# dpmerrell/PathMatFac.jl

Measured on AMD Instinct MI355X. Metric: fit_iters_per_sec, higher is better.
Workload: dtype f32; 1 GPU; fit! epoch on synthetic 200000x50000 matrix (D stored as f32), K=64, Gaussian loss, group-reg X (32 groups) + featureset-ARD Y, adam; rows sharded over 1 GPU(s); full_model=False, M=200000, N=50000, K=64, rows_per_gpu=200000, optimizer=adam, parallelism=single GPU, rccl_ranks=0, collectives_issued=0, column_chunks=1

## Files before the change

### pathmatfac.jl_amd/csrc/pmf_common.h

```cpp
#ifndef PMF_COMMON_H
#define PMF_COMMON_H
#include <hip/hip_runtime.h>

#include <cstdint>
#include <type_traits>
#include <unordered_map>

#include "../../include/pmf_hip.h"

int pmf_fail(const char *fmt, ...);
#define HIPCHK(x)                                                                                    \
  do {                                                                                               \
    hipError_t e_ = (x);                                                                             \
    if (e_ != hipSuccess) return pmf_fail("%s failed: %s (%s:%d)", #x, hipGetErrorString(e_), __FILE__, __LINE__); \
  } while (0)
#define PMFCHK(x)          \
  do {                     \
    int r_ = (x);          \
    if (r_ < 0) return r_; \
  } while (0)

typedef std::unordered_map<const void *, size_t> PmfDynLds;
int pmf_ensure_dyn_lds(PmfDynLds *cache, const void *kern, size_t lds);

// ... 42 lines not shown
  int32_t nbs_shift;
  int32_t n_bv;
  double *loss_partial;
  int64_t M, N;
  int32_t n_cseg;
  int32_t want_gx, want_gy;
  unsigned long long *stamps;
  int32_t dbg;
  const ViewDesc *views;
  const char *Xsb, *Ysb;
  int32_t ct0;
  float *gx_part;
  const int32_t *piece_base;
  int64_t gx_slot_stride;
  const float *sb_scale_x, *sb_scale_y;
};

__device__ __forceinline__ int pmf_rowmap(int r, int h) { return (r & 3) + 8 * (r >> 2) + 4 * h; }
__device__ __forceinline__ bool pmf_finite(float y) { return fabsf(y) <= 3.402823466e38f; }

__host__ __device__ __forceinline__ int pmf_meta_kind(int meta) { return meta & 3; }
__host__ __device__ __forceinline__ int pmf_meta_view(int meta) { return (meta >> 2) - 1; }
__host__ __device__ __forceinline__ int64_t pmf_view_index(const ViewDesc &vd, int64_t j, int b) { return (j - vd.c0) * vd.nb + b; }
__host__ __device__ __forceinline__ int64_t pmf_btab_index(const ViewDesc &vd, int64_t j, int b) { return vd.tab_off + pmf_view_index(vd, j, b); }
__device__ __forceinline__ int pmf_row_batch(const int32_t *bor, int64_t M, int v, int64_t i) { return v >= 0 ? bor[(int64_t)v * M + i] : -1; }
__device__ __forceinline__ float2 pmf_batch_dt(const ViewDesc &vd, const float2 *btab, int64_t j, int b) {
  return b >= 0 ? btab[pmf_btab_index(vd, j, b)] : make_float2(1.f, 0.f);
}

__device__ __forceinline__ void pmf_noise(int kind, float z, float y, float w, float &l, float &g) {
// ... 294 lines not shown
```

### pathmatfac.jl_amd/csrc/pmf_ctx.h

```cpp
#ifndef PMF_CTX_H
#define PMF_CTX_H
#include <hip/hip_runtime.h>

#include <algorithm>
#include <chrono>
#include <cmath>
#include <cstdarg>
#include <cstdio>
#include <cstdlib>
#include <cstring>
#include <string>
#include <unordered_map>
#include <vector>

#include "pmf_common.h"

struct ParamBuf {
  float *p = nullptr, *g = nullptr, *acc = nullptr, *mom = nullptr;
  float *wq = nullptr, *cq = nullptr;
  float *wl1 = nullptr;
  int64_t n = 0;
  float bp1 = 0.f, bp2 = 0.f;
};

// ... 42 lines not shown
  int64_t n = 0, V = 0;
  float p = 1.f;
  std::vector<int64_t> h_voff;
  int64_t *voff = nullptr;
  int64_t *aa_rp = nullptr, *ab_rp = nullptr, *abt_rp = nullptr, *bb_rp = nullptr;
  int32_t *aa_col = nullptr, *ab_col = nullptr, *abt_col = nullptr, *bb_col = nullptr;
  float *aa_val = nullptr, *ab_val = nullptr, *abt_val = nullptr, *bb_val = nullptr;
  float *u = nullptr;
  float *work = nullptr;
  float *PT = nullptr;
  float *grad = nullptr;
  int32_t *iters = nullptr;
  double *uloss = nullptr;
  int rb = 1;
  int64_t vmax = 0;
};

struct pmf_ctx {
  int device = 0;
  hipStream_t stream = nullptr;
  bool own_stream = true;
  int n_cu = 256;
  int64_t M = 0, N = 0;
  int K = 0, Kp = 0, KB = 0;
  void *D = nullptr;
  bool own_D = false;
  int64_t D_M = 0, D_Npad = 0, nRB = 0;
  uint32_t *tflags = nullptr;
  int64_t tflags_cap = 0;
  bool tflags_valid = false;
// ... 39 lines not shown
  std::vector<uint8_t> h_kind;
  std::vector<int64_t> noise_s1, noise_e1;
  std::vector<WorkSplit> splits;
  int n_chunks_req = 0;
  float *gx_part = nullptr;
  size_t gx_part_cap = 0;
  int32_t *gx_off = nullptr, *gx_idx = nullptr;
  int64_t gx_serial = -1;
  int64_t split_serial = 0;
  Comm comm;
  int last_chunks = 1;
  hipEvent_t ev_host = nullptr;
  int64_t kind_version = 0;
  float *gy_slabs = nullptr;
  size_t gy_slabs_cap = 0;
  int precision = PMF_PREC_F32;
  char *xsb = nullptr, *ysb = nullptr;
  size_t xsb_cap = 0, ysb_cap = 0;
  float *sb8_scale = nullptr;
  uint32_t *sb8_max = nullptr;
  int64_t sb_launches = 0;
  int64_t loss_cap = 0;
  int64_t n_macro = 0;
  double *reg_partial = nullptr;
  double *d_loss = nullptr;
  double *h_loss = nullptr;
  std::vector<std::pair<hipEvent_t, hipEvent_t>> ev_pool;
  size_t ev_used = 0;
  double kernel_ms_sum = 0.0;
  int64_t kernel_launches = 0;
// ... 30 lines not shown
    HIPCHK(hipFree(*p));
    *p = nullptr;
  }
  if (n == 0) n = 1;
  HIPCHK(hipMalloc((void **)p, n * sizeof(T)));
  if (zero) PMFCHK(memset_now(*p, 0, n * sizeof(T)));
  return 0;
}
template <typename T>
static void dev_free(T **p) {
  if (*p) (void)hipFree(*p);
  *p = nullptr;
}

template <typename T>
struct DevBuf {
  T *p = nullptr;
  DevBuf() = default;
  DevBuf(const DevBuf &) = delete;
  DevBuf &operator=(const DevBuf &) = delete;
  ~DevBuf() { if (p) (void)hipFree(p); }
  int alloc(size_t n) {
    HIPCHK(hipMalloc((void **)&p, std::max<size_t>(n, 1) * sizeof(T)));
    return 0;
  }
};
template <typename T>
struct PinnedBuf {
  T *p = nullptr;
  PinnedBuf() = default;
  PinnedBuf(const PinnedBuf &) = delete;
  PinnedBuf &operator=(const PinnedBuf &) = delete;
  ~PinnedBuf() { if (p) (void)hipHostFree(p); }
  int alloc(size_t n) {
    HIPCHK(hipHostMalloc((void **)&p, std::max<size_t>(n, 1) * sizeof(T)));
    return 0;
  }
};

__device__ __forceinline__ double block_reduce_sum(double v, double *sh) {
#pragma unroll
  for (int off = 32; off > 0; off >>= 1) v += __shfl_xor(v, off, 64);
// ... 29 lines not shown
  const float b = 1.f + (0.5f / be) * (p * p);
  lacc += (double)(scale * (0.5f + al) * logf(b));
  g += scale * ((al + 0.5f) * p / (b * be));
}

int ctx_bind(pmf_ctx *c);
int ensure_dyn_lds(pmf_ctx *c, const void *kern, size_t lds);
int check_ready(pmf_ctx *c);
int harvest_events(pmf_ctx *c);
int epoch_open(pmf_ctx *c, const pmf_fit_opts *o);
int epoch_layer_pass(pmf_ctx *c, const pmf_fit_opts *o, bool with_loss);
FusedGeom fused_geometry(pmf_ctx *c, bool want_gx, bool want_gy, bool allow_chunks);
int prepare_fused_pass(pmf_ctx *c, const FusedGeom &g, bool want_gx, bool want_gy);
int launch_fused_chunk(pmf_ctx *c, const FusedGeom &g, int s, bool want_gx, bool want_gy);
struct PassExtent { const char *name; int64_t need, cap; };
constexpr int PMF_PASS_EXTENTS = 10;
int fused_pass_extents(pmf_ctx *c, const FusedGeom &g, bool want_gx, bool want_gy, PassExtent *out);
int check_pass_extents(const PassExtent *e, int n);
int guard_fused_pass(pmf_ctx *c, const FusedGeom &g, bool want_gx, bool want_gy);
int step_param_range(pmf_ctx *c, int which, int64_t e0, int64_t n, bool do_step, bool use_reg, int reg_slot, int *reg_count,
                     int max_blocks, bool advance);
int step_param(pmf_ctx *c, int which, bool do_step, bool use_reg, int reg_slot, int *reg_count);
int step_layers(pmf_ctx *c, const pmf_fit_opts *o, int *reg_count);
int launch_loss_reduce(pmf_ctx *c, const RegCounts &rc, int mask);
void step_args_xy(pmf_ctx *c, int which, StepArgs *s);
int eval_full_loss(pmf_ctx *c, double out[4]);
int eval_data_grads(pmf_ctx *c);
int stats_pass_check(pmf_ctx *c);
int stats_pass(pmf_ctx *c, int use_factors, bool want_cols, bool want_batch, const float **cols, const float **batch);
void lbfgs_free(pmf_ctx *c);
void netreg_free(pmf_ctx *c, int which);
// ... 7 lines not shown
```

### pathmatfac.jl_amd/csrc/pmf_fused.hip.inc

```

template <int KB, int NW, int RBW = 1>
struct FusedCfg {
  static constexpr int Kp = 32 * KB;
  static constexpr int KpS = Kp + 4;
  static constexpr int SLAB = 32 * Kp;
  static constexpr int YT = PMF_BN * KpS;
  static constexpr int XP = 32 * KpS;
  static constexpr int TT = (RBW - 1) * 1024;
  static constexpr int FIXED = NW * SLAB + NW * RBW * XP + NW * TT + 8 * PMF_BN + 4;
  static constexpr int LDS_BUDGET = 160 * 1024;
  static constexpr int NYB = (2 * YT + FIXED) * 4 + 8 * NW <= LDS_BUDGET ? 2 : 1;
  static constexpr size_t lds_bytes = (sizeof(float) * (NYB * YT + FIXED) + sizeof(double) * NW + 15) / 16 * 16;
  static constexpr size_t lds_batch_extra = PMF_BN * 16 * sizeof(float2) + PMF_PM_BYTES + NW * RBW * 16 * 32;
};

#ifndef PMF_NW4_WAVES
#define PMF_NW4_WAVES 1
#endif
template <int KB, int NW, int RBW, int BMODE, bool MIXED, int GM, bool DB, bool XW = false>
__global__ __launch_bounds__(64 * NW, (NW == 8 ? 2 : PMF_NW4_WAVES)) void pmf_fused_kernel(const FusedArgs a) {
  using Cfg = FusedCfg<KB, NW, RBW>;
  constexpr bool FULL = GM != 3;
  constexpr bool BATCH = BMODE != 0;
  constexpr bool bt_lds = BMODE == 1;
// ... 43 lines not shown
  }
  const int xw_j = 16 * (w & 1) + (lane & 15), xw_k = 16 * (w >> 1) + 4 * (lane >> 4);
  const int xw_e = xw_j * Kp + xw_k;
  const int xw_x = 4 * (lane >> 4) * KpS + 16 * (w >> 1) + (lane & 15);
  int xw_g[4];
  typedef const __attribute__((address_space(3))) float *lds_cptr;
  unsigned xw_xa[4];
#pragma unroll
  for (int u = 0; u < 4; ++u) {
    const int i = 4 * (lane >> 4) + u;
    xw_g[u] = i * 32 + 4 * ((xw_j >> 2) ^ (i & 7)) + (xw_j & 3);
    xw_xa[u] = (unsigned)(uintptr_t)(lds_cptr)(Xs + xw_x + u * KpS);
    if (XW) asm volatile("" : "+v"(xw_xa[u]));
  }

  constexpr bool HOIST = KB == 2 && NW == 8 && RBW == 1 && GM != 3 && (XW || GM != 0 || BMODE == 0);
  unsigned ho_y[2][YV], ho_s[2][YV], ho_c[2], ho_g[2][RV4];
  if (HOIST) {
#pragma unroll
    for (int z = 0; z < 2; ++z) {
      const int ncol = z == 0 || N % BN == 0 ? BN : (int)(N % BN);
#pragma unroll
      for (int q = 0; q < YV; ++q) {
        int e4 = tid + NT * q;
        if (e4 > BN * Kp / 4 - 1) e4 = BN * Kp / 4 - 1;
        int jl = (e4 * 4) / Kp;
        if (jl >= ncol) { jl = ncol - 1; e4 = jl * (Kp / 4); }
        ho_y[z][q] = 16u * e4;
        ho_s[z][q] = 16u * jl;
        asm volatile("" : "+v"(ho_y[z][q]), "+v"(ho_s[z][q]));
      }
      ho_c[z] = 16u * (tid < ncol ? tid : ncol - 1);
      asm volatile("" : "+v"(ho_c[z]));
#pragma unroll
      for (int q = 0; q < RV4; ++q) {
        int e = xw_e;
        if (!XW) {
          const int f = tid + NT * q, ff = f < BN * Kp / 4 ? f : 0;
          e = ((ff % (BN * 8)) / 8) * Kp + 32 * (ff / (BN * 8)) + 4 * (ff % 8);
        }
        ho_g[z][q] = 4u * (e < ncol * Kp ? e : e % Kp);
        asm volatile("" : "+v"(ho_g[z][q]));
      }
    }
  }
  auto ho_at = [](const void *base, unsigned off) { return reinterpret_cast<const char *>(base) + off; };
#ifdef PMF_STAMPS
  unsigned long long st_acc[16] = {0, 0, 0, 0, 0, 0, 0, 0, 0, 0, 0, 0, 0, 0, 0, 0};
  unsigned long long st_prev = __builtin_amdgcn_s_memtime();
  const unsigned long long st_t0 = st_prev, st_r0 = __builtin_amdgcn_s_memrealtime();
#endif
  const int wg = pmf_xcd_wg(blockIdx.x, gridDim.x);
  const int64_t w_begin = a.wg_begin[wg];
  const int64_t w_end = a.wg_begin[wg + 1];
  float *myslab = a.gy_slabs + (int64_t)wg * a.slab_stride;
  const int64_t seg_block = a.n_rp * a.tps;
  double lossacc = 0.0;
  int seg_cur = -1, pidx = 0, t0_first = 0;
  int gx_slot = (GM == 2) ? 0 : a.piece_base[wg];
// ... 27 lines not shown
      for (int q = 0; q < XV; ++q) {
        const int e4 = lane + 64 * q;
        const int il = (e4 * 4) / Kp;
        const int64_t ir = row0[rb] + il < M ? row0[rb] + il : M - 1;
        xv0[rb][q] = *reinterpret_cast<const float4 *>(a.X + ir * Kp + (e4 * 4) % Kp);
      }
    }
    f32x16 gx[RBW][KB];
#pragma unroll
    for (int rb = 0; rb < RBW; ++rb)
#pragma unroll
      for (int kb = 0; kb < KB; ++kb)
#pragma unroll
        for (int r = 0; r < 16; ++r) gx[rb][kb][r] = 0.f;

    auto stage_load_y = [&](int64_t jt, int q, float4 (&yv)[YV], float (&sgv)[YV]) {
      const float *yb = a.Y + jt * Kp;
      const float4 *cb = a.colp + jt;
      const int64_t rem = N - jt;
      if (HOIST) {
        const bool rag = rem < BN;
        yv[q] = *reinterpret_cast<const float4 *>(ho_at(yb, rag ? ho_y[1][q] : ho_y[0][q]));
        sgv[q] = *reinterpret_cast<const float *>(ho_at(cb, rag ? ho_s[1][q] : ho_s[0][q]));
        return;
      }
      const int ncol = rem > BN ? BN : (int)rem;
      int e4 = tid + NT * q;
      if (e4 > BN * Kp / 4 - 1) e4 = BN * Kp / 4 - 1;
      int jl = (e4 * 4) / Kp;
      if (jl >= ncol) { jl = ncol - 1; e4 = jl * (Kp / 4); }
      yv[q] = *reinterpret_cast<const float4 *>(yb + e4 * 4);
      sgv[q] = cb[jl].x;
    };
    auto stage_load_c = [&](int64_t jt, float4 &cv) {
      const float4 *cb = a.colp + jt;
      const int64_t rem = N - jt;
      if (HOIST) {
        cv = *reinterpret_cast<const float4 *>(ho_at(cb, rem < BN ? ho_c[1] : ho_c[0]));
        return;
      }
      const int ncol = rem > BN ? BN : (int)rem;
      cv = cb[tid < ncol ? tid : ncol - 1];
    };
    auto stage_load = [&](int64_t jt, float4 (&yv)[YV], float (&sgv)[YV], float4 &cv) {
#pragma unroll
      for (int q = 0; q < YV; ++q) stage_load_y(jt, q, yv, sgv);
      stage_load_c(jt, cv);
    };
    auto stage_store = [&](int ybuf, int cbuf, int64_t jt, const float4 (&yv)[YV], const float (&sgv)[YV], const float4 &cv) {
      float *Yn = Ys + ybuf * Cfg::YT;
      const int64_t rem = N - jt;
      const int ncol = rem > BN ? BN : (int)rem;
#pragma unroll
      for (int q = 0; q < YV; ++q) {
        const int e4 = tid + NT * q;
        if (e4 < BN * Kp / 4) {
          const int jl = (e4 * 4) / Kp, kf = (e4 * 4) % Kp;
          const float sg = jl < ncol ? sgv[q] : 0.f;
          *reinterpret_cast<float4 *>(Yn + jl * KpS + kf) = make_float4(yv[q].x * sg, yv[q].y * sg, yv[q].z * sg, yv[q].w * sg);
        }
      }
      asm volatile("" ::"v"(cv.x), "v"(cv.y), "v"(cv.z), "v"(cv.w));
      if (tid < BN) {
        const bool livec = tid < ncol;
        Csg[cbuf * BN + tid] = livec ? cv.x : 0.f;
        Cmu[cbuf * BN + tid] = livec ? cv.y : 0.f;
        Cw[cbuf * BN + tid] = livec ? cv.z : 0.f;
        Cmt[cbuf * BN + tid] = livec ? __float_as_int(cv.w) : 3;
        if (MIXED) {
          const int kd = __float_as_int(cv.w) & 3;
          const unsigned m0 = (unsigned)__ballot(!livec || kd == 0), m1 = (unsigned)__ballot(!livec || kd == 1),
                         m2 = (unsigned)__ballot(!livec || kd == 2);
          if (tid == 0) Ck[cbuf] = m0 == 0xffffffffu ? 0 : (m1 == 0xffffffffu ? 1 : (m2 == 0xffffffffu ? 2 : 3));
        }
        if (bt_lds) {
          const int vw = (__float_as_int(cv.w) >> 2) - 1;
          const int vw0 = __builtin_amdgcn_readfirstlane(vw);
          const unsigned mv = (unsigned)__ballot(!livec || vw == vw0);
          if (tid == 0) Ck[2 + cbuf] = mv == 0xffffffffu ? vw0 : -2;
        }
      }
    };
    auto bt_e = [&](int q) { return (tid & 31) * 16 + (tid >> 5) + (NT / 32) * q; };
// ... 3 lines not shown
      Btd[o] = dt.x;
      Btt[o] = dt.y + mu;
    };
    float4 gold[RV4];
    PmfDTile<DB> dcur[RBW];
    constexpr int DCH = PmfDTile<DB>::NCH;
    auto slab_map = [&](int q, int &so, int &e) -> bool {
      const int f = tid + NT * q;
      const bool in = f < BN * Kp / 4;
      const int ff = in ? f : 0;
      so = 4 * ff;
      e = ((ff % (BN * 8)) / 8) * Kp + 32 * (ff / (BN * 8)) + 4 * (ff % 8);
      return in;
    };
    auto slab_prefetch_one = [&](int64_t jt, int q) {
      const float *sb = myslab + jt * Kp;
      const int64_t rem = N - jt;
      if (HOIST) {
        gold[q] = pmf_load_stream(reinterpret_cast<const float4 *>(ho_at(sb, rem < BN ? ho_g[1][q] : ho_g[0][q])));
        return;
      }
      const int nel = (rem > BN ? BN : (int)rem) * Kp;
      int so, e;
      if (XW) e = xw_e;
      else slab_map(q, so, e);
      gold[q] = pmf_load_stream(reinterpret_cast<const float4 *>(sb + (e < nel ? e : (e % Kp))));
    };
    auto forward_reduce = [&](f32x16 (&acc)[RBW], int ybuf, int cbuf, bool do_red, int64_t jt_red) {
      const int cb0 = cbuf * BN + 4 * h;
#pragma unroll
      for (int r = 0; r < 16; ++r) {
        const float m0 = BATCH ? 0.f : Cmu[cb0 + (r & 3) + 8 * (r >> 2)];
#pragma unroll
        for (int rb = 0; rb < RBW; ++rb) acc[rb][r] = m0;
      }
      const float4 *yr = reinterpret_cast<const float4 *>(Ys + ybuf * Cfg::YT + l31 * KpS + h * (Kp / 2));
      const float4 *xr[RBW];
      float4 yv = yr[0], xv[RBW];
#pragma unroll
      for (int rb = 0; rb < RBW; ++rb) {
        xr[rb] = reinterpret_cast<const float4 *>(Xw[rb] + l31 * KpS + h * (Kp / 2));
// ... 35 lines not shown
        for (int rb = 0; rb < RBW; ++rb) acc[rb] = __builtin_amdgcn_mfma_f32_32x32x2f32(yv.y, xv[rb].y, acc[rb], 0, 0, 0);
#pragma unroll
        for (int rb = 0; rb < RBW; ++rb) acc[rb] = __builtin_amdgcn_mfma_f32_32x32x2f32(yv.z, xv[rb].z, acc[rb], 0, 0, 0);
#pragma unroll
        for (int rb = 0; rb < RBW; ++rb) acc[rb] = __builtin_amdgcn_mfma_f32_32x32x2f32(yv.w, xv[rb].w, acc[rb], 0, 0, 0);
        yv = yn;
#pragma unroll
        for (int rb = 0; rb < RBW; ++rb) xv[rb] = xn[rb];
        __builtin_amdgcn_sched_barrier(0);
      }
      if (do_red && (FULL || !(dbg & 8))) {
#pragma unroll
        for (int rb = 0; rb < RBW; ++rb) {
          dcur[rb].touch();
        }
        const int64_t rem = N - jt_red;
        const int nel = (rem > BN ? BN : (int)rem) * Kp;
        float *sb = myslab + jt_red * Kp;
#pragma unroll
        for (int q = 0; q < RV4; ++q) {
          float4 v = racc[q];
          const float sgj = Csg[(cbuf ^ 1) * BN + eo[q] / Kp];
          v.x *= sgj; v.y *= sgj; v.z *= sgj; v.w *= sgj;
          if (!slab_first) { v.x += gold[q].x; v.y += gold[q].y; v.z += gold[q].z; v.w += gold[q].w; }
          if (in[q] && eo[q] < nel) pmf_store_stream(reinterpret_cast<float4 *>(sb + eo[q]), v);
        }
      }
    };

    bool rows_in[RBW];
    int rb_u[RBW];
    uint32_t tflag[RBW];
#pragma unroll
    for (int rb = 0; rb < RBW; ++rb) {
      const int rb_raw = __builtin_amdgcn_readfirstlane((int)(row0[rb] >> 5));
      rows_in[rb] = rb_raw < a.nRB;
      rb_u[rb] = rows_in[rb] ? rb_raw : (int)a.nRB - 1;
      tflag[rb] = a.tflags[(col_begin >> 5) * a.nRB + rb_u[rb]];
#pragma unroll
      for (int q = 0; q < DCH; ++q) dcur[rb].load(a.D, (col_begin >> 5) * a.nRB + rb_u[rb], lane, q);
    }
    {
      float4 yv[YV], cv;
      float sgv[YV];
      stage_load(col_begin, yv, sgv, cv);
#pragma unroll
      for (int rb = 0; rb < RBW; ++rb)
#pragma unroll
        for (int q = 0; q < XV; ++q) {
          const int e4 = lane + 64 * q;
          const int il = (e4 * 4) / Kp, kf = (e4 * 4) % Kp;
          *reinterpret_cast<float4 *>(Xw[rb] + il * KpS + kf) = row0[rb] + il < M ? xv0[rb][q] : make_float4(0.f, 0.f, 0.f, 0.f);
        }
      stage_store(0, 0, col_begin, yv, sgv, cv);
      if (bt_lds) {
#pragma unroll
        for (int q = 0; q < NBT; ++q) {
          const int e = bt_e(q);
          bt_store(e, pmf_bt_entry(a, a.pm + rp * a.n_bv * 16, col_begin, e, pmf_bt_view(a, col_begin, e)), bt_mu(col_begin, e));
        }
        if (tid < a.n_bv * 16) Pm[tid] = a.pm[rp * a.n_bv * 16 + tid];
        if (h == 0)
#pragma unroll
          for (int rb = 0; rb < RBW; ++rb)
            for (int v = 0; v < a.n_bv; ++v) Bw0[rb * 512 + v * 32 + l31] = a.row_slot[(int64_t)v * M + irow_c[rb]];
      }
    }
    __syncthreads();

    f32x16 acc[RBW];
    forward_reduce(acc, 0, 0, false, 0);

    for (int t = 0; t < ntiles; ++t) {
      const int par = t & 1;
      const int cur = NYB == 2 ? par : 0, nxt = NYB == 2 ? (par ^ 1) : 0;
      const int64_t j0 = col_begin + (int64_t)t * BN;
      const float *Yc = Ys + cur * Cfg::YT;
      const bool have_next = (t + 1 < ntiles);
      const int cb0 = par * BN + 4 * h;
      float4 ynext[YV], cnext;
      float2 btn[NBT];
      float btm[NBT];
      int btv[NBT];
      float sgnext[YV];
      PMF_STAMP(0);
      const float xw_sg = XW ? Csg[par * BN + xw_j] : 0.f;

      float lsum = 0.f;
      const int tkind = MIXED ? __builtin_amdgcn_readfirstlane(Ck[par]) : 0;
      const int tview = bt_lds ? __builtin_amdgcn_readfirstlane(Ck[2 + par]) : -1;
      float lnorm = 0.f;
      auto epi_reg = [&](int rb, int r, float dl, float th, float wj, int kmode, bool fast) __attribute__((always_inline)) {
        if (dbg & 4) return;
        float z = acc[rb][r];
        if (BATCH) z = fmaf(z, dl, th);
        float y = dcur[rb].get(r);
        if (kmode == PMF_NOISE_NORMAL) {
          if (!fast) y = (pmf_finite(y) && row_ok[rb]) ? y : z;
          const float d = z - y, g = wj * d;
// ... 45 lines not shown
      };
      const float4 *cw4 = reinterpret_cast<const float4 *>(Cw + cb0);
      auto f4get = [](const float4 &v, int u) { return u == 0 ? v.x : (u == 1 ? v.y : (u == 2 ? v.z : v.w)); };

      const int64_t jn = have_next ? j0 + BN : j0;
      constexpr int NOTH = YV + 1 + RV4 + (BATCH ? NBT : 0);
      constexpr int NVM = NOTH + (DCH + 1) * RBW;
      bool tile_fast[RBW];
#pragma unroll
      for (int rb = 0; rb < RBW; ++rb) tile_fast[rb] = rows_in[rb] && tflag[rb] != 0;
      auto vmem_op = [&](int i) {
        if (i == 0 && bt_lds) {
#pragma unroll
          for (int q = 0; q < NBT; ++q) btv[q] = pmf_bt_view(a, jn, bt_e(q));
        }
        if (i < YV) stage_load_y(jn, i, ynext, sgnext);
        else if (i == YV) stage_load_c(jn, cnext);
        else if (i < YV + 1 + RV4) { if (want_gy) slab_prefetch_one(j0, i - YV - 1); }
        else if (i < NOTH) {
          const int q = i - YV - 1 - RV4;
          if (bt_lds) { btn[q] = pmf_bt_entry(a, Pm, jn, bt_e(q), btv[q]); btm[q] = bt_mu(jn, bt_e(q)); }
        }
        else if (i < NVM) {
          const int rb = (i - NOTH) / (DCH + 1), q = (i - NOTH) % (DCH + 1);
          if (q < DCH) {
            if (FULL || !(dbg & 2)) dcur[rb].load(a.D, (jn >> 5) * a.nRB + rb_u[rb], lane, q);
          } else {
            tflag[rb] = a.tflags[(jn >> 5) * a.nRB + rb_u[rb]];
          }
        }
      };
// ... 39 lines not shown
          else if (!MIXED || tkind == 0) { if (BATCH && tile_fast[rb]) epi_all(PMF_NOISE_NORMAL, true, true); else epi_all(PMF_NOISE_NORMAL, true, false); }
          else if (tkind == 1) epi_all(PMF_NOISE_BERNOULLI, true, false);
          else if (tkind == 2) epi_all(PMF_NOISE_POISSON, true, false);
          else epi_all(3, true, false);
        }
        if (want_gy) {
#pragma unroll
          for (int c4 = 0; c4 < 4; ++c4)
            *reinterpret_cast<float4 *>((XW ? Sl + (par * NW + w) * 1024 : T[rb]) + l31 * 32 + 4 * ((2 * c4 + h) ^ (l31 & 7))) =
                make_float4(acc[rb][4 * c4], acc[rb][4 * c4 + 1], acc[rb][4 * c4 + 2], acc[rb][4 * c4 + 3]);
        }
      }
      PMF_STAMP(1);
      if (want_gx) {
        float bq[3][KB];
#pragma unroll
        for (int s0 = 0; s0 < 2; ++s0) {
          const float *yp = Yc + pmf_rowmap(s0, h) * KpS + l31;
#pragma unroll
          for (int kb = 0; kb < KB; ++kb) bq[s0][kb] = yp[32 * kb];
        }
        __builtin_amdgcn_sched_barrier(0);
#pragma unroll
        for (int s = 0; s < 16; ++s) {
          if (s + 2 < 16) {
            const float *yp = Yc + pmf_rowmap(s + 2, h) * KpS + l31;
#pragma unroll
            for (int kb = 0; kb < KB; ++kb) bq[(s + 2) % 3][kb] = yp[32 * kb];
          }
          if (s < NVM) vmem_op(s);
#pragma unroll
          for (int rb = 0; rb < RBW; ++rb)
#pragma unroll
            for (int kb = 0; kb < KB; ++kb)
              gx[rb][kb] = __builtin_amdgcn_mfma_f32_32x32x2f32(acc[rb][s], bq[s % 3][kb], gx[rb][kb], 0, 0, 0);
          __builtin_amdgcn_sched_barrier(0);
        }
#pragma unroll
        for (int i = 16; i < NVM; ++i) vmem_op(i);
      } else if (GM != 2) {
#pragma unroll
        for (int i = 0; i < NVM; ++i) vmem_op(i);
      }
// ... 26 lines not shown
        if (!(dbg & 32)) {
#pragma unroll
          for (int kb = 0; kb < KB; ++kb)
#pragma unroll
            for (int r = 0; r < 16; ++r) Sw[kb * 1024 + pmf_rowmap(r, h) * 32 + l31] = gy[kb][r];
        } else {
          f32x16 keep = gy[0];
#pragma unroll
          for (int kb = 1; kb < KB; ++kb) keep += gy[kb];
          asm volatile("" ::"v"(keep));
        }
      }

      PMF_STAMP(4);
      if (NYB == 1) __syncthreads();
      stage_store(nxt, par ^ 1, jn, ynext, sgnext, cnext);
      PMF_STAMP(5);
      __syncthreads();
      PMF_STAMP(6);

      if (bt_lds) {
#pragma unroll
        for (int q = 0; q < NBT; ++q) bt_store(bt_e(q), btn[q], btm[q]);
      }
      slab_first = pidx == 0 || (pidx == 1 && ti0 + t < t0_first);
      if (XW) {
        typedef float f32x4 __attribute__((ext_vector_type(4)));
        constexpr int XW_RING = 8, XW_AHEAD = 6;
        const float *Gp = Sl + par * (NW * 1024);
        float xa[XW_RING], xb[XW_RING];
        auto xw_read = [&](int q) __attribute__((always_inline)) {
// ... 4 lines not shown
            xb[(q + hi) % XW_RING] = Gp[p * 1024 + xw_g[u] + 512 * hi];
          }
        };
#pragma unroll
        for (int q = 0; q < XW_AHEAD; q += 2) xw_read(q);
        f32x4 gy0 = {0.f, 0.f, 0.f, 0.f}, gy1 = {0.f, 0.f, 0.f, 0.f};
        __builtin_amdgcn_sched_barrier(0);
#pragma unroll
        for (int q = 0; q < 8 * NW; q += 2) {
          if (q + XW_AHEAD < 8 * NW) xw_read(q + XW_AHEAD);
          gy0 = __builtin_amdgcn_mfma_f32_16x16x4f32(xa[q % XW_RING], xb[q % XW_RING], gy0, 0, 0, 0);
          gy1 = __builtin_amdgcn_mfma_f32_16x16x4f32(xa[(q + 1) % XW_RING], xb[(q + 1) % XW_RING], gy1, 0, 0, 0);
          __builtin_amdgcn_sched_barrier(0);
        }
        dcur[0].touch();
        const int64_t rem = N - j0;
        const int nel = (rem > BN ? BN : (int)rem) * Kp;
        float4 v = make_float4((gy0[0] + gy1[0]) * xw_sg, (gy0[1] + gy1[1]) * xw_sg, (gy0[2] + gy1[2]) * xw_sg, (gy0[3] + gy1[3]) * xw_sg);
        if (!slab_first) { v.x += gold[0].x; v.y += gold[0].y; v.z += gold[0].z; v.w += gold[0].w; }
        if (xw_e < nel) pmf_store_stream(reinterpret_cast<float4 *>(myslab + j0 * Kp + xw_e), v);
        PMF_STAMP(4);
        forward_reduce(acc, nxt, par ^ 1, false, 0);
        PMF_STAMP(8);
        if (bt_lds) __syncthreads();
        PMF_STAMP(9);
      } else {
        if (FULL || have_next) forward_reduce(acc, nxt, par ^ 1, want_gy && !(dbg & 1), j0);
        else if (want_gy && !(dbg & 1)) { f32x16 dummy[RBW]; forward_reduce(dummy, nxt, par ^ 1, true, j0); }
        PMF_STAMP(8);
        if ((GM != 1 || bt_lds) && !(dbg & 16)) __syncthreads();
        PMF_STAMP(9);
      }
    }
    if (XW && !bt_lds) __syncthreads();

// ... 31 lines not shown
```

### pathmatfac.jl_amd/csrc/pmf_hip.hip

```cpp
#include "pmf_ctx.h"

static thread_local std::string g_err;
int pmf_fail(const char *fmt, ...) {
  char buf[1024];
  va_list ap;
  va_start(ap, fmt);
  vsnprintf(buf, sizeof(buf), fmt, ap);
  va_end(ap);
  g_err = buf;
  return -1;
}
extern "C" const char *pmf_last_error(void) { return g_err.c_str(); }
extern "C" int pmf_version(void) { return 1; }


int ctx_bind(pmf_ctx *c) {
  if (!c) return pmf_fail("null context");
  HIPCHK(hipSetDevice(c->device));
  return 0;
}

int memset_now(void *p, int v, size_t bytes) {
  HIPCHK(hipMemset(p, v, bytes));
  HIPCHK(hipStreamSynchronize(nullptr));
// ... 32 lines not shown
  HIPCHK(hipMalloc(&c->scratch, bytes));
  c->scratch_bytes = bytes;
  return 0;
}

__global__ void k_fill(float *p, int64_t n, float v) {
  for (int64_t e = blockIdx.x * (int64_t)blockDim.x + threadIdx.x; e < n; e += (int64_t)gridDim.x * blockDim.x) p[e] = v;
}

__global__ void k_prepare(const float *logsigma, const float *mu, const float *colw, const int32_t *colmeta,
                          float4 *colp, int64_t N, const float *logdelta, const float *theta, float2 *btab,
                          int64_t nbt) {
  const int64_t e = blockIdx.x * (int64_t)blockDim.x + threadIdx.x;
  if (e < N) colp[e] = make_float4(expf(logsigma[e]), mu[e], colw[e], __int_as_float(colmeta[e]));
  if (e < nbt) btab[e] = make_float2(expf(logdelta[e]), theta[e]);
}

struct DenseBtabArgs {
  const int32_t *colmeta;
  const float2 *btab;
  float2 *btd;
  uint8_t *colview;
  int64_t N, Npad;
  int32_t nbs_shift;
  ViewDesc views[PMF_MAXV];
};
__global__ void k_dense_btab(const DenseBtabArgs a) {
  const int64_t e = blockIdx.x * (int64_t)blockDim.x + threadIdx.x;
  if (e >= (a.Npad << a.nbs_shift)) return;
  const int64_t j = e >> a.nbs_shift;
// ... 1427 lines not shown
static void chunk_segments(pmf_ctx *c, const FusedGeom &g, int s, int &grid, int64_t &tps, int64_t &n_cseg) {
  const int64_t n_ct = g.nct[s], n_rp = g.n_rp;
  grid = (int)std::min<int64_t>(n_rp * n_ct, (int64_t)g.grid_max);
  const double tiles_per_wg = (double)(n_rp * n_ct) / grid;
  const double a_cost = tiles_per_wg * 8e-6;
  const double b_cost = (double)grid * (double)c->Kp * (double)n_ct * 32.0 * 4.0 / ((double)n_ct * 4e12);
  tps = (int64_t)std::llround(std::sqrt(a_cost / std::max(b_cost, 1e-12)));
  {
    const char *ts = getenv("PMF_TPS_SCALE");
    if (ts) tps = (int64_t)std::llround((double)tps * atof(ts));
  }
  tps = std::max<int64_t>(std::min<int64_t>(8, n_ct), std::min<int64_t>(tps, n_ct));
  n_cseg = std::max<int64_t>(1, n_ct / tps);
}

int prepare_fused_pass(pmf_ctx *c, const FusedGeom &g, bool want_gx, bool want_gy) {
  if (!g.fam) return pmf_fail("unsupported KB=%d", c->KB);
  const FusedFamily &f = *g.fam;
  if ((int)c->splits.size() < g.S) c->splits.resize((size_t)g.S);
  int64_t grid_sum = 0, serial_sum = 0;
  for (int s = 0; s < g.S; ++s) {
    int grid; int64_t tps, n_cseg;
    chunk_segments(c, g, s, grid, tps, n_cseg);
    PMFCHK(compute_work_split(c, c->splits[(size_t)s], grid, g.n_rp, g.ct0[s], g.nct[s], tps, n_cseg, f.kernel != 0));
    grid_sum += grid;
  }
  serial_sum = c->split_serial * PMF_MAX_CHUNKS + g.S;
  PMFCHK(ensure_loss_partials(c, grid_sum));
  const int64_t slab_stride = (int64_t)c->Kp * c->N;
  const size_t gy_need = (size_t)g.grid_max * (size_t)slab_stride + (size_t)PMF_BN * (size_t)c->Kp;
  if (want_gy && gy_need > c->gy_slabs_cap) {
    dev_free(&c->gy_slabs);
    c->gy_slabs_cap = 0;
    PMFCHK(dev_alloc(&c->gy_slabs, gy_need, false));
    c->gy_slabs_cap = gy_need;
  }
  if (want_gx && serial_sum != c->gx_serial) {
    std::vector<std::vector<int32_t>> lists((size_t)g.n_rp);
    int32_t base = 0;
    for (int s = 0; s < g.S; ++s) {
      WorkSplit &ws = c->splits[(size_t)s];
      ws.slot_base = base;
      for (size_t p = 0; p < ws.piece_rp.size(); ++p) lists[(size_t)ws.piece_rp[p]].push_back(base + (int32_t)p);
      std::vector<int32_t> abs(ws.h_piece_base);
// ... 13 lines not shown
    HIPCHK(hipMemcpy(c->gx_idx, idx.data(), sizeof(int32_t) * idx.size(), hipMemcpyHostToDevice));
    c->gx_serial = serial_sum;
  }
  if (want_gx) {
    size_t pieces = 0;
    for (int s = 0; s < g.S; ++s) pieces += c->splits[(size_t)s].piece_rp.size();
    const size_t need = pieces * (size_t)f.BM() * (size_t)c->Kp;
    if (need > c->gx_part_cap) {
      dev_free(&c->gx_part);
      c->gx_part_cap = 0;
      PMFCHK(dev_alloc(&c->gx_part, need, false));
      c->gx_part_cap = need;
    }
  }
  PMFCHK(ensure_tile_flags(c));
  if (f.img != IMG_NONE) {
    size_t xblk = 0, yblk = 0;
    for (const FusedFamily &o : fused_families)
      if (o.img_kb == f.img_kb) { xblk = std::max<size_t>(xblk, o.xblk); yblk = std::max<size_t>(yblk, o.yblk); }
    const size_t xb = ((size_t)c->nRB + PMF_XSB_PAD) * xblk, yb = (size_t)g.n_ct_all * yblk;
    if (xb > c->xsb_cap) { dev_free(&c->xsb); c->xsb_cap = 0; PMFCHK(dev_alloc(&c->xsb, xb, true)); c->xsb_cap = xb; }
    if (yb > c->ysb_cap) { dev_free(&c->ysb); c->ysb_cap = 0; PMFCHK(dev_alloc(&c->ysb, yb, false)); c->ysb_cap = yb; }
    if (f.img == IMG_SB8 && !c->sb8_scale) {
      PMFCHK(dev_alloc(&c->sb8_scale, (size_t)(1 + PMF_MAX_CHUNKS), false));
      PMFCHK(dev_alloc(&c->sb8_max, (size_t)(1 + PMF_MAX_CHUNKS)));
    }
  }
  return 0;
}

int fused_pass_extents(pmf_ctx *c, const FusedGeom &g, bool want_gx, bool want_gy, PassExtent *out) {
  const FusedFamily &f = *g.fam;
  const int64_t Kp = c->Kp, Npad = g.n_ct_all * PMF_BN;
  int64_t pieces = 0, grid_sum = 0, grid_top = 0;
  for (int s = 0; s < g.S; ++s) {
    const WorkSplit &ws = c->splits[(size_t)s];
    pieces += (int64_t)ws.piece_rp.size();
    grid_sum += ws.grid;
    grid_top = std::max<int64_t>(grid_top, ws.grid);
  }
  const bool bt = g.bmode == 1;
  int nbs_shift = 0;
  while ((1 << nbs_shift) < c->nbs) ++nbs_shift;
  const int64_t gx_slot_stride = (int64_t)f.BM() * Kp, slab_stride = Kp * c->N;
  int n = 0;
  out[n++] = {"gx_part", want_gx ? pieces * gx_slot_stride * 4 : 0, (int64_t)c->gx_part_cap * 4};
  out[n++] = {"gy_slabs", want_gy ? ((grid_top - 1) * slab_stride + (f.img == IMG_SB8 ? Npad * Kp : slab_stride)) * 4 : 0,
              (int64_t)c->gy_slabs_cap * 4};
  out[n++] = {"xsb", f.img != IMG_NONE ? (c->nRB + f.nblk - 1) / f.nblk * f.nblk * f.xblk : 0, (int64_t)c->xsb_cap};
  out[n++] = {"ysb", f.img != IMG_NONE ? g.n_ct_all * f.yblk : 0, (int64_t)c->ysb_cap};
  out[n++] = {"btd", bt ? (Npad << nbs_shift) * (int64_t)sizeof(float2) : 0, c->btd_cap * (int64_t)sizeof(float2)};
  out[n++] = {"colview", bt ? Npad : 0, c->colview_cap};
  out[n++] = {"tflags", g.n_ct_all * c->nRB * 4, c->tflags_cap * 4};
  out[n++] = {"loss_partial", grid_sum * 8, c->loss_cap * 8};
  out[n++] = {"pm", bt ? g.n_rp * c->n_bv * 16 : 0, bt ? g.ps->pm_cap : 0};
  out[n++] = {"row_slot", bt ? (int64_t)c->n_bv * c->M : 0, bt ? g.ps->row_slot_cap : 0};
  static_assert(PMF_PASS_EXTENTS == 10, "fused_pass_extents");
  return n;
}
int check_pass_extents(const PassExtent *e, int n) {
  for (int i = 0; i < n; ++i)
    if (e[i].need > e[i].cap)
      return pmf_fail("data pass refused: it addresses %lld bytes of %s, %lld are allocated", (long long)e[i].need, e[i].name,
                      (long long)e[i].cap);
  return 0;
}
int guard_fused_pass(pmf_ctx *c, const FusedGeom &g, bool want_gx, bool want_gy) {
  PassExtent e[PMF_PASS_EXTENTS];
  return check_pass_extents(e, fused_pass_extents(c, g, want_gx, want_gy, e));
}

static int sb8_split(pmf_ctx *c, const FusedFamily &f, const float *src, const float4 *colp, int64_t n, int64_t nblk, int slot,
// ... 22 lines not shown
  if (f.img == IMG_SB4) {
    Sb4SplitArgs s4 = {src, c->colp + c0, c->N - c0, nct, c->Kp, 0, out};
    return pmf_launch_sb4_split(c->stream, s4);
  }
  SbSplitArgs sy = {src, c->colp + c0, c->N - c0, nct, out};
  return f.KB == 1 ? pmf_launch_sb_split_1(c->stream, sy) : pmf_launch_sb_split_2(c->stream, sy);
}

int launch_fused_chunk(pmf_ctx *c, const FusedGeom &g, int s, bool want_gx, bool want_gy) {
  const FusedFamily &f = *g.fam;
  WorkSplit &ws = c->splits[(size_t)s];
  const int grid = ws.grid;
  int grid_dummy; int64_t tiles_per_seg, n_cseg;
  chunk_segments(c, g, s, grid_dummy, tiles_per_seg, n_cseg);
  const int64_t n_ct = g.nct[s], n_rp = g.n_rp;
  const int64_t slab_stride = (int64_t)c->Kp * c->N;
  int64_t loss_off = 0;
  for (int q = 0; q < s; ++q) loss_off += c->splits[(size_t)q].grid;
  FusedArgs a;
  memset(&a, 0, sizeof(a));
  a.tflags = c->tflags;
  a.wg_begin = ws.wg_begin;
  a.D = c->D; a.X = c->P[0].p; a.Y = c->P[1].p; a.gX = c->P[0].g; a.gY = c->P[1].g;
  a.colp = c->colp; a.bor = c->bor; a.btab = c->btab; a.loss_partial = c->loss_partial + loss_off;
  a.btd = g.bmode == 1 ? c->btd : nullptr; a.n_bv = c->n_bv;
  if (g.bmode == 1) {
    a.pm = g.ps->pm; a.row_slot = g.ps->row_slot; a.colview = c->colview;
    a.nbs_shift = 0;
    while ((1 << a.nbs_shift) < c->nbs) ++a.nbs_shift;
  }
  c->last_bmode = g.bmode;
// ... 10 lines not shown
  {
    static unsigned long long *d_stamps = nullptr;
    if (!d_stamps) HIPCHK(hipMalloc((void **)&d_stamps, sizeof(unsigned long long) * 16 * 8 * 1024));
    HIPCHK(hipMemsetAsync(d_stamps, 0, sizeof(unsigned long long) * 16 * 8 * 1024, c->stream));
    a.stamps = d_stamps;
    g_stamps = d_stamps;
  }
#endif
  a.views = c->d_views;
  const bool batch = c->n_bv > 0;
  if (f.img != IMG_NONE) {
    if (s == 0) PMFCHK(sb_split_x(c, f));
    PMFCHK(sb_split_y(c, f, g.ct0[s], n_ct, s));
    a.Xsb = c->xsb; a.Ysb = c->ysb;
    if (f.img == IMG_SB8) { a.sb_scale_x = c->sb8_scale; a.sb_scale_y = c->sb8_scale + 1 + s; }
  }
  if (c->ev_used == c->ev_pool.size()) {
    if (c->ev_pool.size() >= 4096) {
      HIPCHK(hipStreamSynchronize(c->stream));
      harvest_events(c);
    } else {
      hipEvent_t e0, e1;
      HIPCHK(hipEventCreate(&e0));
      HIPCHK(hipEventCreate(&e1));
      c->ev_pool.emplace_back(e0, e1);
    }
  }
  auto &ev = c->ev_pool[c->ev_used++];
  HIPCHK(hipEventRecord(ev.first, c->stream));
  c->last_kernel = f.kernel;
// ... 582 lines not shown
```

Baseline: 31.43 iters/s.

## Prescale Y into padded image buffer to drop ragged-edge logic in fused kernel

```diff
diff --git a/pathmatfac.jl_amd/csrc/pmf_common.h b/pathmatfac.jl_amd/csrc/pmf_common.h
--- a/pathmatfac.jl_amd/csrc/pmf_common.h
+++ b/pathmatfac.jl_amd/csrc/pmf_common.h
@@ -80,6 +80,8 @@
   const int32_t *piece_base;
   int64_t gx_slot_stride;
   const float *sb_scale_x, *sb_scale_y;
+  const float *yimg;
+  const float4 *colpad;
 };
 
 __device__ __forceinline__ int pmf_rowmap(int r, int h) { return (r & 3) + 8 * (r >> 2) + 4 * h; }
diff --git a/pathmatfac.jl_amd/csrc/pmf_ctx.h b/pathmatfac.jl_amd/csrc/pmf_ctx.h
--- a/pathmatfac.jl_amd/csrc/pmf_ctx.h
+++ b/pathmatfac.jl_amd/csrc/pmf_ctx.h
@@ -80,6 +80,28 @@
   double *uloss = nullptr;
   int rb = 1;
   int64_t vmax = 0;
+};
+
+template <typename T>
+struct DevBuf {
+  T *p = nullptr;
+  size_t cap = 0;
+  DevBuf() = default;
+  DevBuf(const DevBuf &) = delete;
+  DevBuf &operator=(const DevBuf &) = delete;
+  ~DevBuf() { if (p) (void)hipFree(p); }
+  int alloc(size_t n) {
+    HIPCHK(hipMalloc((void **)&p, std::max<size_t>(n, 1) * sizeof(T)));
+    cap = n;
+    return 0;
+  }
+  int reserve(size_t n) {
+    if (p && n <= cap) return 0;
+    if (p) (void)hipFree(p);
+    p = nullptr;
+    cap = 0;
+    return alloc(n);
+  }
 };
 
 struct pmf_ctx {
@@ -149,6 +171,8 @@
   int64_t kind_version = 0;
   float *gy_slabs = nullptr;
   size_t gy_slabs_cap = 0;
+  DevBuf<float> yimg;
+  DevBuf<float4> colpad;
   int precision = PMF_PREC_F32;
   char *xsb = nullptr, *ysb = nullptr;
   size_t xsb_cap = 0, ysb_cap = 0;
@@ -209,18 +233,6 @@
 }
 
 template <typename T>
-struct DevBuf {
-  T *p = nullptr;
-  DevBuf() = default;
-  DevBuf(const DevBuf &) = delete;
-  DevBuf &operator=(const DevBuf &) = delete;
-  ~DevBuf() { if (p) (void)hipFree(p); }
-  int alloc(size_t n) {
-    HIPCHK(hipMalloc((void **)&p, std::max<size_t>(n, 1) * sizeof(T)));
-    return 0;
-  }
-};
-template <typename T>
 struct PinnedBuf {
   T *p = nullptr;
   PinnedBuf() = default;
@@ -280,7 +292,7 @@
 int prepare_fused_pass(pmf_ctx *c, const FusedGeom &g, bool want_gx, bool want_gy);
 int launch_fused_chunk(pmf_ctx *c, const FusedGeom &g, int s, bool want_gx, bool want_gy);
 struct PassExtent { const char *name; int64_t need, cap; };
-constexpr int PMF_PASS_EXTENTS = 10;
+constexpr int PMF_PASS_EXTENTS = 12;
 int fused_pass_extents(pmf_ctx *c, const FusedGeom &g, bool want_gx, bool want_gy, PassExtent *out);
 int check_pass_extents(const PassExtent *e, int n);
 int guard_fused_pass(pmf_ctx *c, const FusedGeom &g, bool want_gx, bool want_gy);
diff --git a/pathmatfac.jl_amd/csrc/pmf_fused.hip.inc b/pathmatfac.jl_amd/csrc/pmf_fused.hip.inc
--- a/pathmatfac.jl_amd/csrc/pmf_fused.hip.inc
+++ b/pathmatfac.jl_amd/csrc/pmf_fused.hip.inc
@@ -81,35 +81,36 @@
     if (XW) asm volatile("" : "+v"(xw_xa[u]));
   }
 
+#ifndef PMF_G2B
+#define PMF_G2B 1
+#endif
+  constexpr bool G2B = KB == 2 && PMF_G2B != 0;
+  unsigned g2_ya[KB];
+#pragma unroll
+  for (int kb = 0; kb < KB; ++kb) {
+    g2_ya[kb] = (unsigned)(uintptr_t)(lds_cptr)(Ys + 4 * h * KpS + 32 * kb + l31);
+    if (G2B) asm volatile("" : "+v"(g2_ya[kb]));
+  }
+
   constexpr bool HOIST = KB == 2 && NW == 8 && RBW == 1 && GM != 3 && (XW || GM != 0 || BMODE == 0);
-  unsigned ho_y[2][YV], ho_s[2][YV], ho_c[2], ho_g[2][RV4];
-  if (HOIST) {
-#pragma unroll
-    for (int z = 0; z < 2; ++z) {
-      const int ncol = z == 0 || N % BN == 0 ? BN : (int)(N % BN);
-#pragma unroll
-      for (int q = 0; q < YV; ++q) {
-        int e4 = tid + NT * q;
-        if (e4 > BN * Kp / 4 - 1) e4 = BN * Kp / 4 - 1;
-        int jl = (e4 * 4) / Kp;
-        if (jl >= ncol) { jl = ncol - 1; e4 = jl * (Kp / 4); }
-        ho_y[z][q] = 16u * e4;
-        ho_s[z][q] = 16u * jl;
-        asm volatile("" : "+v"(ho_y[z][q]), "+v"(ho_s[z][q]));
-      }
-      ho_c[z] = 16u * (tid < ncol ? tid : ncol - 1);
-      asm volatile("" : "+v"(ho_c[z]));
-#pragma unroll
-      for (int q = 0; q < RV4; ++q) {
-        int e = xw_e;
-        if (!XW) {
-          const int f = tid + NT * q, ff = f < BN * Kp / 4 ? f : 0;
-          e = ((ff % (BN * 8)) / 8) * Kp + 32 * (ff / (BN * 8)) + 4 * (ff % 8);
-        }
-        ho_g[z][q] = 4u * (e < ncol * Kp ? e : e % Kp);
-        asm volatile("" : "+v"(ho_g[z][q]));
-      }
+  unsigned ho_y[YV], ho_c, ho_g[RV4];
+#pragma unroll
+  for (int q = 0; q < YV; ++q) {
+    const int e4 = tid + NT * q;
+    ho_y[q] = 16u * (e4 < BN * Kp / 4 ? e4 : BN * Kp / 4 - 1);
+    if (HOIST) asm volatile("" : "+v"(ho_y[q]));
+  }
+  ho_c = 16u * (tid & (BN - 1));
+  if (HOIST) asm volatile("" : "+v"(ho_c));
+#pragma unroll
+  for (int q = 0; q < RV4; ++q) {
+    int e = xw_e;
+    if (!XW) {
+      const int f = tid + NT * q, ff = f < BN * Kp / 4 ? f : 0;
+      e = ((ff % (BN * 8)) / 8) * Kp + 32 * (ff / (BN * 8)) + 4 * (ff % 8);
     }
+    ho_g[q] = 4u * e;
+    if (HOIST) asm volatile("" : "+v"(ho_g[q]));
   }
   auto ho_at = [](const void *base, unsigned off) { return reinterpret_cast<const char *>(base) + off; };
 #ifdef PMF_STAMPS
@@ -167,59 +168,32 @@
 #pragma unroll
         for (int r = 0; r < 16; ++r) gx[rb][kb][r] = 0.f;
 
-    auto stage_load_y = [&](int64_t jt, int q, float4 (&yv)[YV], float (&sgv)[YV]) {
-      const float *yb = a.Y + jt * Kp;
-      const float4 *cb = a.colp + jt;
-      const int64_t rem = N - jt;
-      if (HOIST) {
-        const bool rag = rem < BN;
-        yv[q] = *reinterpret_cast<const float4 *>(ho_at(yb, rag ? ho_y[1][q] : ho_y[0][q]));
-        sgv[q] = *reinterpret_cast<const float *>(ho_at(cb, rag ? ho_s[1][q] : ho_s[0][q]));
-        return;
-      }
-      const int ncol = rem > BN ? BN : (int)rem;
-      int e4 = tid + NT * q;
-      if (e4 > BN * Kp / 4 - 1) e4 = BN * Kp / 4 - 1;
-      int jl = (e4 * 4) / Kp;
-      if (jl >= ncol) { jl = ncol - 1; e4 = jl * (Kp / 4); }
-      yv[q] = *reinterpret_cast<const float4 *>(yb + e4 * 4);
-      sgv[q] = cb[jl].x;
-    };
-    auto stage_load_c = [&](int64_t jt, float4 &cv) {
-      const float4 *cb = a.colp + jt;
-      const int64_t rem = N - jt;
-      if (HOIST) {
-        cv = *reinterpret_cast<const float4 *>(ho_at(cb, rem < BN ? ho_c[1] : ho_c[0]));
-        return;
-      }
-      const int ncol = rem > BN ? BN : (int)rem;
-      cv = cb[tid < ncol ? tid : ncol - 1];
-    };
-    auto stage_load = [&](int64_t jt, float4 (&yv)[YV], float (&sgv)[YV], float4 &cv) {
-#pragma unroll
-      for (int q = 0; q < YV; ++q) stage_load_y(jt, q, yv, sgv);
+    auto stage_load_y = [&](int64_t jt, int q, float4 (&yv)[YV]) {
+      yv[q] = *reinterpret_cast<const float4 *>(ho_at(a.yimg + jt * Kp, ho_y[q]));
+    };
+    auto stage_load_c = [&](int64_t jt, float4 &cv) { cv = *reinterpret_cast<const float4 *>(ho_at(a.colpad + jt, ho_c)); };
+    auto stage_load = [&](int64_t jt, float4 (&yv)[YV], float4 &cv) {
+#pragma unroll
+      for (int q = 0; q < YV; ++q) stage_load_y(jt, q, yv);
       stage_load_c(jt, cv);
     };
-    auto stage_store = [&](int ybuf, int cbuf, int64_t jt, const float4 (&yv)[YV], const float (&sgv)[YV], const float4 &cv) {
+    auto stage_store = [&](int ybuf, int cbuf, const float4 (&yv)[YV], const float4 &cv) {
       float *Yn = Ys + ybuf * Cfg::YT;
-      const int64_t rem = N - jt;
-      const int ncol = rem > BN ? BN : (int)rem;
 #pragma unroll
       for (int q = 0; q < YV; ++q) {
         const int e4 = tid + NT * q;
         if (e4 < BN * Kp / 4) {
           const int jl = (e4 * 4) / Kp, kf = (e4 * 4) % Kp;
-          const float sg = jl < ncol ? sgv[q] : 0.f;
-          *reinterpret_cast<float4 *>(Yn + jl * KpS + kf) = make_float4(yv[q].x * sg, yv[q].y * sg, yv[q].z * sg, yv[q].w * sg);
+          *reinterpret_cast<float4 *>(Yn + jl * KpS + kf) = yv[q];
         }
       }
       asm volatile("" ::"v"(cv.x), "v"(cv.y), "v"(cv.z), "v"(cv.w));
       if (tid < BN) {
-        const bool livec = tid < ncol;
-        Csg[cbuf * BN + tid] = livec ? cv.x : 0.f;
-        Cmu[cbuf * BN + tid] = livec ? cv.y : 0.f;
-        Cw[cbuf * BN + tid] = livec ? cv.z : 0.f;
-        Cmt[cbuf * BN + tid] = livec ? __float_as_int(cv.w) : 3;
+        Csg[cbuf * BN + tid] = cv.x;
+        Cmu[cbuf * BN + tid] = cv.y;
+        Cw[cbuf * BN + tid] = cv.z;
+        Cmt[cbuf * BN + tid] = __float_as_int(cv.w);
+        const bool livec = (__float_as_int(cv.w) & 3) != 3;
         if (MIXED) {
           const int kd = __float_as_int(cv.w) & 3;
           const unsigned m0 = (unsigned)__ballot(!livec || kd == 0), m1 = (unsigned)__ballot(!livec || kd == 1),
@@ -253,17 +227,13 @@
       return in;
     };
     auto slab_prefetch_one = [&](int64_t jt, int q) {
-      const float *sb = myslab + jt * Kp;
-      const int64_t rem = N - jt;
-      if (HOIST) {
-        gold[q] = pmf_load_stream(reinterpret_cast<const float4 *>(ho_at(sb, rem < BN ? ho_g[1][q] : ho_g[0][q])));
-        return;
-      }
-      const int nel = (rem > BN ? BN : (int)rem) * Kp;
-      int so, e;
-      if (XW) e = xw_e;
-      else slab_map(q, so, e);
-      gold[q] = pmf_load_stream(reinterpret_cast<const float4 *>(sb + (e < nel ? e : (e % Kp))));
+      gold[q] = pmf_load_stream(reinterpret_cast<const float4 *>(ho_at(myslab + jt * Kp, ho_g[q])));
+    };
+    auto slab_add_old = [&](float4 &v, const float4 &o) __attribute__((always_inline)) {
+      if (!slab_first) {
+        if (KB == 2) asm volatile("" : "+v"(v.x), "+v"(v.y), "+v"(v.z), "+v"(v.w));
+        v.x += o.x; v.y += o.y; v.z += o.z; v.w += o.w;
+      }
     };
     auto forward_reduce = [&](f32x16 (&acc)[RBW], int ybuf, int cbuf, bool do_red, int64_t jt_red) {
       const int cb0 = cbuf * BN + 4 * h;
@@ -329,16 +299,14 @@
         for (int rb = 0; rb < RBW; ++rb) {
           dcur[rb].touch();
         }
-        const int64_t rem = N - jt_red;
-        const int nel = (rem > BN ? BN : (int)rem) * Kp;
         float *sb = myslab + jt_red * Kp;
 #pragma unroll
         for (int q = 0; q < RV4; ++q) {
           float4 v = racc[q];
           const float sgj = Csg[(cbuf ^ 1) * BN + eo[q] / Kp];
           v.x *= sgj; v.y *= sgj; v.z *= sgj; v.w *= sgj;
-          if (!slab_first) { v.x += gold[q].x; v.y += gold[q].y; v.z += gold[q].z; v.w += gold[q].w; }
-          if (in[q] && eo[q] < nel) pmf_store_stream(reinterpret_cast<float4 *>(sb + eo[q]), v);
+          slab_add_old(v, gold[q]);
+          if (in[q]) pmf_store_stream(reinterpret_cast<float4 *>(sb + eo[q]), v);
         }
       }
     };
@@ -357,8 +325,7 @@
     }
     {
       float4 yv[YV], cv;
-      float sgv[YV];
-      stage_load(col_begin, yv, sgv, cv);
+      stage_load(col_begin, yv, cv);
 #pragma unroll
       for (int rb = 0; rb < RBW; ++rb)
 #pragma unroll
@@ -367,7 +334,7 @@
           const int il = (e4 * 4) / Kp, kf = (e4 * 4) % Kp;
           *reinterpret_cast<float4 *>(Xw[rb] + il * KpS + kf) = row0[rb] + il < M ? xv0[rb][q] : make_float4(0.f, 0.f, 0.f, 0.f);
         }
-      stage_store(0, 0, col_begin, yv, sgv, cv);
+      stage_store(0, 0, yv, cv);
       if (bt_lds) {
 #pragma unroll
         for (int q = 0; q < NBT; ++q) {
@@ -397,7 +364,6 @@
       float2 btn[NBT];
       float btm[NBT];
       int btv[NBT];
-      float sgnext[YV];
       PMF_STAMP(0);
       const float xw_sg = XW ? Csg[par * BN + xw_j] : 0.f;
 
@@ -473,7 +439,7 @@
 #pragma unroll
           for (int q = 0; q < NBT; ++q) btv[q] = pmf_bt_view(a, jn, bt_e(q));
         }
-        if (i < YV) stage_load_y(jn, i, ynext, sgnext);
+        if (i < YV) stage_load_y(jn, i, ynext);
         else if (i == YV) stage_load_c(jn, cnext);
         else if (i < YV + 1 + RV4) { if (want_gy) slab_prefetch_one(j0, i - YV - 1); }
         else if (i < NOTH) {
@@ -543,19 +509,27 @@
       PMF_STAMP(1);
       if (want_gx) {
         float bq[3][KB];
+        unsigned g2_y[KB];
+#pragma unroll
+        for (int kb = 0; kb < KB; ++kb) {
+          g2_y[kb] = g2_ya[kb] + 4u * (unsigned)(cur * Cfg::YT);
+          if (G2B) asm volatile("" : "+v"(g2_y[kb]));
+        }
+        auto g2_b = [&](int s, int kb) -> float {
+          if (G2B) return *(lds_cptr)(uintptr_t)(g2_y[kb] + 4u * (unsigned)(pmf_rowmap(s, 0) * KpS));
+          return Yc[pmf_rowmap(s, h) * KpS + l31 + 32 * kb];
+        };
 #pragma unroll
         for (int s0 = 0; s0 < 2; ++s0) {
-          const float *yp = Yc + pmf_rowmap(s0, h) * KpS + l31;
-#pragma unroll
-          for (int kb = 0; kb < KB; ++kb) bq[s0][kb] = yp[32 * kb];
+#pragma unroll
+          for (int kb = 0; kb < KB; ++kb) bq[s0][kb] = g2_b(s0, kb);
         }
         __builtin_amdgcn_sched_barrier(0);
 #pragma unroll
         for (int s = 0; s < 16; ++s) {
           if (s + 2 < 16) {
-            const float *yp = Yc + pmf_rowmap(s + 2, h) * KpS + l31;
-#pragma unroll
-            for (int kb = 0; kb < KB; ++kb) bq[(s + 2) % 3][kb] = yp[32 * kb];
+#pragma unroll
+            for (int kb = 0; kb < KB; ++kb) bq[(s + 2) % 3][kb] = g2_b(s + 2, kb);
           }
           if (s < NVM) vmem_op(s);
 #pragma unroll
@@ -612,7 +586,7 @@
 
       PMF_STAMP(4);
       if (NYB == 1) __syncthreads();
-      stage_store(nxt, par ^ 1, jn, ynext, sgnext, cnext);
+      stage_store(nxt, par ^ 1, ynext, cnext);
       PMF_STAMP(5);
       __syncthreads();
       PMF_STAMP(6);
@@ -647,11 +621,9 @@
           __builtin_amdgcn_sched_barrier(0);
         }
         dcur[0].touch();
-        const int64_t rem = N - j0;
-        const int nel = (rem > BN ? BN : (int)rem) * Kp;
         float4 v = make_float4((gy0[0] + gy1[0]) * xw_sg, (gy0[1] + gy1[1]) * xw_sg, (gy0[2] + gy1[2]) * xw_sg, (gy0[3] + gy1[3]) * xw_sg);
-        if (!slab_first) { v.x += gold[0].x; v.y += gold[0].y; v.z += gold[0].z; v.w += gold[0].w; }
-        if (xw_e < nel) pmf_store_stream(reinterpret_cast<float4 *>(myslab + j0 * Kp + xw_e), v);
+        slab_add_old(v, gold[0]);
+        pmf_store_stream(reinterpret_cast<float4 *>(reinterpret_cast<char *>(myslab + j0 * Kp) + ho_g[0]), v);
         PMF_STAMP(4);
         forward_reduce(acc, nxt, par ^ 1, false, 0);
         PMF_STAMP(8);
diff --git a/pathmatfac.jl_amd/csrc/pmf_hip.hip b/pathmatfac.jl_amd/csrc/pmf_hip.hip
--- a/pathmatfac.jl_amd/csrc/pmf_hip.hip
+++ b/pathmatfac.jl_amd/csrc/pmf_hip.hip
@@ -70,6 +70,21 @@
   const int64_t e = blockIdx.x * (int64_t)blockDim.x + threadIdx.x;
   if (e < N) colp[e] = make_float4(expf(logsigma[e]), mu[e], colw[e], __int_as_float(colmeta[e]));
   if (e < nbt) btab[e] = make_float2(expf(logdelta[e]), theta[e]);
+}
+
+__global__ void k_y_image(const float *__restrict__ Y, const float4 *__restrict__ colp, float *__restrict__ yimg,
+                          float4 *__restrict__ colpad, int64_t e0, int64_t n4, int64_t N, int Kp) {
+  const int64_t t = blockIdx.x * (int64_t)blockDim.x + threadIdx.x;
+  if (t >= n4) return;
+  const int64_t e = e0 + 4 * t, j = e / Kp;
+  float4 v = make_float4(0.f, 0.f, 0.f, 0.f), cp = make_float4(0.f, 0.f, 0.f, __int_as_float(3));
+  if (j < N) {
+    cp = colp[j];
+    const float4 y = *reinterpret_cast<const float4 *>(Y + e);
+    v = make_float4(y.x * cp.x, y.y * cp.x, y.z * cp.x, y.w * cp.x);
+  }
+  *reinterpret_cast<float4 *>(yimg + e) = v;
+  if (e == j * Kp) colpad[j] = cp;
 }
 
 struct DenseBtabArgs {
@@ -1527,6 +1542,10 @@
   n_cseg = std::max<int64_t>(1, n_ct / tps);
 }
 
+static int64_t fused_slab_stride(const pmf_ctx *c, const FusedGeom &g) {
+  return (int64_t)c->Kp * (g.fam->img == IMG_NONE ? g.n_ct_all * PMF_BN : c->N);
+}
+
 int prepare_fused_pass(pmf_ctx *c, const FusedGeom &g, bool want_gx, bool want_gy) {
   if (!g.fam) return pmf_fail("unsupported KB=%d", c->KB);
   const FusedFamily &f = *g.fam;
@@ -1540,7 +1559,7 @@
   }
   serial_sum = c->split_serial * PMF_MAX_CHUNKS + g.S;
   PMFCHK(ensure_loss_partials(c, grid_sum));
-  const int64_t slab_stride = (int64_t)c->Kp * c->N;
+  const int64_t slab_stride = fused_slab_stride(c, g);
   const size_t gy_need = (size_t)g.grid_max * (size_t)slab_stride + (size_t)PMF_BN * (size_t)c->Kp;
   if (want_gy && gy_need > c->gy_slabs_cap) {
     dev_free(&c->gy_slabs);
@@ -1584,6 +1603,10 @@
     }
   }
   PMFCHK(ensure_tile_flags(c));
+  if (f.img == IMG_NONE) {
+    PMFCHK(c->yimg.reserve((size_t)g.n_ct_all * PMF_BN * (size_t)c->Kp));
+    PMFCHK(c->colpad.reserve((size_t)g.n_ct_all * PMF_BN));
+  }
   if (f.img != IMG_NONE) {
     size_t xblk = 0, yblk = 0;
     for (const FusedFamily &o : fused_families)
@@ -1612,20 +1635,22 @@
   const bool bt = g.bmode == 1;
   int nbs_shift = 0;
   while ((1 << nbs_shift) < c->nbs) ++nbs_shift;
-  const int64_t gx_slot_stride = (int64_t)f.BM() * Kp, slab_stride = Kp * c->N;
+  const int64_t gx_slot_stride = (int64_t)f.BM() * Kp, slab_stride = fused_slab_stride(c, g);
   int n = 0;
   out[n++] = {"gx_part", want_gx ? pieces * gx_slot_stride * 4 : 0, (int64_t)c->gx_part_cap * 4};
   out[n++] = {"gy_slabs", want_gy ? ((grid_top - 1) * slab_stride + (f.img == IMG_SB8 ? Npad * Kp : slab_stride)) * 4 : 0,
               (int64_t)c->gy_slabs_cap * 4};
   out[n++] = {"xsb", f.img != IMG_NONE ? (c->nRB + f.nblk - 1) / f.nblk * f.nblk * f.xblk : 0, (int64_t)c->xsb_cap};
   out[n++] = {"ysb", f.img != IMG_NONE ? g.n_ct_all * f.yblk : 0, (int64_t)c->ysb_cap};
+  out[n++] = {"yimg", f.img == IMG_NONE ? Npad * Kp * 4 : 0, (int64_t)c->yimg.cap * 4};
+  out[n++] = {"colpad", f.img == IMG_NONE ? Npad * 16 : 0, (int64_t)c->colpad.cap * 16};
   out[n++] = {"btd", bt ? (Npad << nbs_shift) * (int64_t)sizeof(float2) : 0, c->btd_cap * (int64_t)sizeof(float2)};
   out[n++] = {"colview", bt ? Npad : 0, c->colview_cap};
   out[n++] = {"tflags", g.n_ct_all * c->nRB * 4, c->tflags_cap * 4};
   out[n++] = {"loss_partial", grid_sum * 8, c->loss_cap * 8};
   out[n++] = {"pm", bt ? g.n_rp * c->n_bv * 16 : 0, bt ? g.ps->pm_cap : 0};
   out[n++] = {"row_slot", bt ? (int64_t)c->n_bv * c->M : 0, bt ? g.ps->row_slot_cap : 0};
-  static_assert(PMF_PASS_EXTENTS == 10, "fused_pass_extents");
+  static_assert(PMF_PASS_EXTENTS == 12, "fused_pass_extents");
   return n;
 }
 int check_pass_extents(const PassExtent *e, int n) {
@@ -1678,7 +1703,7 @@
   int grid_dummy; int64_t tiles_per_seg, n_cseg;
   chunk_segments(c, g, s, grid_dummy, tiles_per_seg, n_cseg);
   const int64_t n_ct = g.nct[s], n_rp = g.n_rp;
-  const int64_t slab_stride = (int64_t)c->Kp * c->N;
+  const int64_t slab_stride = fused_slab_stride(c, g);
   int64_t loss_off = 0;
   for (int q = 0; q < s; ++q) loss_off += c->splits[(size_t)q].grid;
   FusedArgs a;
@@ -1719,6 +1744,11 @@
     PMFCHK(sb_split_y(c, f, g.ct0[s], n_ct, s));
     a.Xsb = c->xsb; a.Ysb = c->ysb;
     if (f.img == IMG_SB8) { a.sb_scale_x = c->sb8_scale; a.sb_scale_y = c->sb8_scale + 1 + s; }
+  } else {
+    const int64_t e0 = g.ct0[s] * PMF_BN * c->Kp, n4 = n_ct * PMF_BN * c->Kp / 4;
+    k_y_image<<<nblocks(n4, 256), 256, 0, c->stream>>>(c->P[1].p, c->colp, c->yimg.p, c->colpad.p, e0, n4, c->N, c->Kp);
+    HIPCHK(hipGetLastError());
+    a.yimg = c->yimg.p; a.colpad = c->colpad.p;
   }
   if (c->ev_used == c->ev_pool.size()) {
     if (c->ev_pool.size() >= 4096) {
```

Result: no change. 31.55 iters/s, median of 6 (+0.4%).
